# AlanConfluent/flink

Hardware: AMD Instinct MI355X
Metric: records/sec aggregated (1M-key tumbling SUM) (higher is better)
Workload: dtype int64

## Files before the change

flink_amd/csrc/engine.hip:

```cpp
#include <hip/hip_runtime.h>
#include <hipcub/device/device_radix_sort.hpp>
#include <hipcub/device/device_scan.hpp>

#include <algorithm>
#include <cstdio>
#include <cstdlib>
#include <cstring>
#include <map>
#include <set>
#include <string>
#include <vector>

#include "../../include/flink_amd.h"
#include "java_math.h"
#include "dec_view.h"

#define LONG_MIN_J ((int64_t)0x8000000000000000LL)
#define LONG_MAX_J ((int64_t)0x7fffffffffffffffLL)

namespace {

#include "ingest.inc"


// ... 1793 lines not shown
    if (rel2slot) {
        uint8_t* code = (uint8_t*)(rel2slot + kRelCap);
        uint8_t* fresh = code + kRelCap;
        for (int32_t i = t; i < kRelCap; i += nt) {
            const int32_t j = i - tab.lo;
            const bool in = j >= 0 && j < tab.n;
            rel2slot[i] = in ? tab.slot[j] : -1;
            code[i] = in ? tab.code[j] : kCodeSlow;
            fresh[i] = in ? tab.fresh[j] : (uint8_t)0;
        }
    }
    if (t == 0) {
        st->error = 0; st->spill_n = 0; st->want_n = 0; st->key_full = 0;
        st->rows = 0;
        st->dropped = 0; st->late_fire = 0; st->max_q = 0; st->min_q = ~0ull; st->ovf_n = 0; st->strag_n = 0; st->wide_n = 0;
    }
    for (int32_t i = t; i < nwant; i += nt) want[i] = 0ull;
    for (int32_t i = t; i < nbcnt; i += nt) bcnt[i] = 0u;
}

struct SlotList { int32_t n, id[15]; };
__global__ void reset_slots_kernel(unsigned long long* const* slot_base, const int32_t* list, SlotList inl, int64_t stride,
                                   int32_t* touched, const EngineConst* __restrict__ cp) {
    const EngineConst& c = *cp;
    const int32_t sid = inl.n ? inl.id[blockIdx.y] : list[blockIdx.y];
    const int32_t slot = sid < 0 ? ~sid : sid;
    if (sid < 0) {
        if (blockIdx.x == 0 && threadIdx.x == 0) touched[slot] = 0;
        return;
    }
// ... 228 lines not shown
    bool sparse = false;
    bool red = false;
    unsigned long long* d_rk = nullptr;
    int32_t* d_iota = nullptr;
    int64_t iota_cap = 0;
    int64_t iota_n = 0;
    bool iota_pending = false, iota_ran = false;
    int32_t* d_rslots = nullptr;
    int64_t rslots_cap = 0;
    int64_t rk_cap = 0;
    int64_t red_seq_base = 0;
    SpState* sp = nullptr;
    int32_t opt_pre = -1, opt_mp = -1, opt_narrow = -1, opt_cells = -1;
    int32_t opt_variant = 0;
    int64_t stragglers = 0;
    bool rows_zero = false;
    int64_t fused_fires = 0;
    int64_t reset_launches = 0;
    int32_t push_epoch = 0;
    unsigned long long* d_rsum = nullptr;
    bool rs_valid = false;
    int64_t rs_q0 = 0;
    int32_t rs_u0 = 0, rs_epoch = 0;
    int32_t rs_k = 4;
    bool rs_on = true;
    int64_t rs_used = 0;
    int64_t opt_out_min = 0;
    bool opt_partials_v1 = false;
    int32_t opt_profile = 0;
    void* d_mf = nullptr;
// ... 905 lines not shown
        e->d_bval[0] = e->d_bval[1] = nullptr;
        const int64_t ent = capb * e->np * kSub + 8 * kMaxPart;
        HIPCHK(e, hipMalloc(&e->d_bkey, (e->nv == 1 ? 12 : 8) * ent));
        HIPCHK(e, hipMalloc(&e->d_brel, 2 * ent));
        for (int v = 0; v < e->nv; ++v) HIPCHK(e, hipMalloc(&e->d_bval[v], 8 * ent));
        e->capb = capb;
    }
    if (need_bn && !e->d_bn) HIPCHK(e, hipMalloc(&e->d_bn, 2 * (e->capb * e->np * kSub + 8 * kMaxPart)));
    if (!e->d_bcnt) {
        HIPCHK(e, hipMalloc(&e->d_bcnt, sizeof(uint32_t) * kMaxPart * kSub));
        HIPCHK(e, hipMalloc(&e->d_rel2slot, (sizeof(int32_t) + 2) * kRelCap));
    }
    return FWA_OK;
}

static int print_phase_profile(fwa_engine* e, const char* tag, hipEvent_t a, hipEvent_t b, int nb, int nph) {
    HIPCHK(e, hipStreamSynchronize(e->stream));
    float ms = 0.f;
    HIPCHK(e, hipEventElapsedTime(&ms, a, b));
    std::vector<long long> hp(8 * (size_t)nb);
    HIPCHK(e, hipMemcpy(hp.data(), e->d_prof, sizeof(long long) * 8 * nb, hipMemcpyDeviceToHost));
    double tot[8] = {0};
    int bmax = 0;
    long long bsum_max = -1;
    for (int blk = 0; blk < nb; ++blk) {
        long long bs = 0;
        for (int k = 0; k < nph; ++k) { tot[k] += (double)hp[blk * 8 + k] / nb; bs += hp[blk * 8 + k]; }
        if (bs > bsum_max) { bsum_max = bs; bmax = blk; }
    }
    fprintf(stderr, "[%s] kernel %.3f ms; per-block avg cycles:", tag, ms);
    for (int k = 0; k < nph; ++k) fprintf(stderr, " %.0f", tot[k]);
    fprintf(stderr, " | slowest block %d:", bmax);
    for (int k = 0; k < nph; ++k) fprintf(stderr, " %lld", hp[bmax * 8 + k]);
    fprintf(stderr, "\n");
    return FWA_OK;
}

static int ensure_sort_tmp(fwa_engine* e, size_t bytes);
static int push_v2(fwa_engine* e, IngestArgs& a, bool* ran) {
    *ran = false;
    int layout = 0;
    if (e->nacc_comb == 1) layout = 2;
    else if (e->nacc_comb == 2 && e->ec.acc_kind[1] == ACC_ADD_I64) {
        for (int j = 0; j < e->cfg.num_aggs; ++j)
            if (e->ec.agg[j].acc == 1 && e->ec.agg[j].vslot == 0) layout = 1;
    }
    const bool pre_ok = (layout == 2 && e->nv == 0) || (layout == 1 && e->nv == 1 && e->vsize[0] == 8);
    if (a.pcount && (!pre_ok || e->cfg.nullable_cols || e->opt_partials_v1)) return FWA_OK;
// ... 77 lines not shown
    pa.b_val0 = e->d_bval[0];
    pa.b_val1 = e->d_bval[1];
    pa.b_cnt = e->d_bcnt;
    pa.capb = e->capb;
    pa.trash = (uint64_t)e->capb * e->np * kSub;
    pa.spill_cap = e->spill_cap;
    pa.part_bits = e->part_bits;
    pa.np = e->np;
    pa.sub_major = (e->opt_variant & 4) ? 0 : 1;
    pa.iota1 = e->ec.red_iota && e->nv == 2 && e->vcol[1] == kIotaCol && e->vsize[1] == 4 && !(e->opt_variant & 16);
    if (e->iota_pending && !pa.iota1) { int rc = ensure_iota(e); if (rc) return rc; }
    for (int v = 0; v < 2; ++v) { pa.vcol[v] = e->vcol[v]; pa.vsize[v] = e->vsize[v]; }
    pa.dropidx = a.pcount ? nullptr : a.dropidx;
    for (int c = 0; c < FWA_MAX_COLS; ++c) { pa.nulls[c] = a.nulls[c]; pa.any_null |= a.nulls[c] != nullptr; }
    pa.st = e->d_st;
    if (e->opt_profile && !e->d_prof) HIPCHK(e, hipMalloc(&e->d_prof, sizeof(long long) * 8 * kMaxPart));
    pa.prof = e->opt_profile ? e->d_prof : nullptr;
    HIPCHK(e, hipEventRecord(e->ev[4], e->stream));
    const int threads = 1024;
    const int items = e->nv == 2 ? 4 : (e->nv == 1 ? 6 : 8);
    const int64_t tile = (int64_t)items * threads;
    const int grid = (int)std::max<int64_t>(1, std::min<int64_t>((a.n + tile - 1) / tile, 256));
    const int vw = (e->vsize[0] == 8 ? 1 : 0) | (e->vsize[1] == 8 ? 2 : 0);
    const bool kg_all = e->cfg.kg_start == 0 && e->cfg.kg_end == e->cfg.max_parallelism - 1 &&
                        e->cfg.key_kind != FWA_KEY_GROUP_PREFIXED;
    const int kgm = kg_all ? 0 : (e->cfg.key_kind == FWA_KEY_PREHASHED ? 2 : 1);
    auto al16 = [](const void* q) { return q == nullptr || ((uintptr_t)q & 15) == 0; };
    const bool w16 = kgm == 0 && al16(pa.keys) && al16(pa.ts) &&
                     (e->nv == 0 || ((uintptr_t)pa.cols[pa.vcol[0]] & ((e->vsize[0] == 8) ? 15 : 7)) == 0);
    const bool narrow = e->opt_narrow != 0 && (e->opt_narrow == 1 || e->narrow) && layout == 1 && e->nv == 1 &&
                        (vw & 1) && w16 && !pre && !a.pcount;
// ... 56 lines not shown
#define FWA_C3_IT0 4
#endif
#ifndef FWA_C3_IT1
#define FWA_C3_IT1 4
#endif
#ifndef FWA_C3_IT2
#define FWA_C3_IT2 3
#endif
#ifndef FWA_C3_NIT
#define FWA_C3_NIT 6
#endif
#ifndef FWA_MP_IT
#define FWA_MP_IT 2
#endif
    constexpr int TH3 = FWA_C3_TH;
#define C3M(IT, NV, LY, PR) do { if (mp) combine3_kernel<FWA_MP_IT, 2, NV, TH3, LY, PR, 1><<<e->np, TH3, lds3, e->stream>>>(ca, e->d_ec); \
        else combine3_kernel<IT, 2, NV, TH3, LY, PR, 0><<<e->np, TH3, lds3, e->stream>>>(ca, e->d_ec); } while (0)
#define C3L(IT, NV) do { \
        if (pre && layout == 1) C3M(IT, 1, 1, 1); \
        else if (pre) C3M(IT, 0, 2, 1); \
        else if (layout == 1) C3M(IT, NV, 1, 0); \
        else if (layout == 2) C3M(IT, NV, 2, 0); \
        else C3M(IT, NV, 0, 0); } while (0)
    if (narrow) {
        if (mp) combine3_kernel<FWA_MP_IT, 2, 1, TH3, 1, 0, 1, 1><<<e->np, TH3, lds3, e->stream>>>(ca, e->d_ec);
        else if (TH3 != 1024 || (e->opt_variant & 2)) combine3_kernel<FWA_C3_NIT, 2, 1, TH3, 1, 0, 0, 1><<<e->np, TH3, lds3, e->stream>>>(ca, e->d_ec);
        else combine3_kernel<6, 2, 1, 1024, 1, 0, 0, 1, 3><<<e->np, 1024, lds3, e->stream>>>(ca, e->d_ec);
    } else if (narrow2) {
        if (mp) combine3_kernel<FWA_MP_IT, 2, 2, TH3, 0, 0, 1, 2><<<e->np, TH3, lds3, e->stream>>>(ca, e->d_ec);
        else combine3_kernel<4, 2, 2, TH3, 0, 0, 0, 2><<<e->np, TH3, lds3, e->stream>>>(ca, e->d_ec);
    } else if (e->nv == 0) C3L(FWA_C3_IT0, 0);
    else if (e->nv == 1) C3L(FWA_C3_IT1, 1);
    else C3L(FWA_C3_IT2, 2);
#undef C3L
#undef C3M
    HIPCHK(e, hipGetLastError());
    HIPCHK(e, hipEventRecord(e->ev[7], e->stream));
    e->v2_timing_pending = true;
    if (e->opt_profile) {
        int rc2 = print_phase_profile(e, "aprof", e->ev[6], e->ev[7], e->np, 8);
        if (rc2) return rc2;
    }
    e->ingest_launches++;
    e->ingest_records += a.n;
    *ran = true;
    return FWA_OK;
}

struct KidEq {
    int tb;
    __host__ __device__ bool operator()(unsigned long long x, unsigned long long y) const { return (x >> tb) == (y >> tb); }
};
struct MaxI64 {
    __host__ __device__ int64_t operator()(int64_t x, int64_t y) const { return x > y ? x : y; }
};
// ... 759 lines not shown
        if (rc) return rc;
        if (e->v2_timing_pending) {
            float ms = 0.f;
            HIPCHK(e, hipEventElapsedTime(&ms, e->ev[4], e->ev[5]));
            e->partition_ms += ms;
            e->ingest_ms += ms;
            HIPCHK(e, hipEventElapsedTime(&ms, e->ev[6], e->ev[7]));
            e->combine_ms += ms;
            e->ingest_ms += ms;
            e->v2_timing_pending = false;
        }
        if (!ran_v2 || round > 0) { rc = account_ingest(e); if (rc) return rc; }
        const DevStatus st = *e->h_st;
        if (ran_v2 && round == 0 && (int64_t)st.ovf_n * 64 > n) e->pre = true;
        if (ran_v2 && round == 0 && (int64_t)st.strag_n * 64 > n) e->mp = true;
        if (ran_v2 && round == 0) e->stragglers += st.strag_n;
        if (ran_v2 && round == 0 && e->narrow_used && (int64_t)st.wide_n * 64 > n) e->narrow = false;
        if (st.error) {
            const char* m = st.error == FWA_E_KEYGROUP ? "Key group is not in the owned KeyGroupRange (StateTable.getMapForKeyGroup)"
                          : st.error == FWA_E_TS_MIN ? "Record has Long.MIN_VALUE timestamp (= no timestamp marker)."
                          : st.error == FWA_E_OOM ? (st.key_full ? "key table full: raise fwa_config.key_capacity" : "slice want-set overflow")
                                                  : "device error";
            return fail(e, st.error, m);
        }
        if (st.late_fire) {
            const size_t o = late_idx.size();
            late_idx.resize(o + st.late_fire);
            HIPCHK(e, hipMemcpy(late_idx.data() + o, e->d_late, 4 * (size_t)st.late_fire, hipMemcpyDeviceToHost));
        }
        dropped += (int64_t)st.dropped;
        if (st.max_q) qmax = std::max<int64_t>(qmax, jm::unord_i64(st.max_q));
// ... 1443 lines not shown
        case FWA_OPT_PARTIALS_ONE_PASS: e->opt_partials_v1 = value > 0; return FWA_OK;
        case FWA_OPT_SP_TABLE: case FWA_OPT_SP_FMAX: case FWA_OPT_SP_BUDGET: return sp_set_option(e, option, value);
        case FWA_OPT_PROFILE: e->opt_profile = value > 0 ? 1 : 0; return FWA_OK;
        case FWA_OPT_INGEST_VARIANT: e->opt_variant = (int32_t)std::max<int64_t>(0, value); return FWA_OK;
        case FWA_OPT_SLIDE_CARRIED: e->rs_on = value != 0; e->rs_valid = false; return FWA_OK;
        case FWA_OPT_FIRE_PARTIALS: e->opt_fire_partials = value != 0 ? 1 : 0; return FWA_OK;
        case FWA_OPT_DEC_WRAP_NULL: e->opt_dec_wrap_null = value != 0 ? 1 : 0; return FWA_OK;
        case FWA_OPT_DISTINCT_SLOTS:
            if (!e->dist) return fail(e, FWA_E_UNSUPPORTED, "FWA_OPT_DISTINCT_SLOTS: no COUNT(DISTINCT) aggregate");
            if (e->dist->d_tab) return fail(e, FWA_E_STATE, "FWA_OPT_DISTINCT_SLOTS: before the first push");
            if (value < 64 || (value & (value - 1)) || value > ((int64_t)1 << 40))
                return fail(e, FWA_E_ARG, "FWA_OPT_DISTINCT_SLOTS: a power of two >= 64");
            e->dist->first_slots = value;
            return FWA_OK;
        case FWA_OPT_DISTINCT_LIVE: case FWA_OPT_DISTINCT_REBUILDS: case FWA_OPT_STRAGGLERS: case FWA_OPT_KEY_TABLE_DIGEST:
        case FWA_OPT_DISTINCT_INDEX_US: case FWA_OPT_DISTINCT_COUNT_US: case FWA_OPT_DISTINCT_COUNT_STEPS:
            return fail(e, FWA_E_ARG, "read-only option");
        default: return fail(e, FWA_E_ARG, "unknown option");
    }
}

int fwa_get_option(const fwa_engine* e, int32_t option, int64_t* value) {
    if (!e || !value) return FWA_E_ARG;
    auto eff = [](int32_t opt, bool adaptive_on) -> int64_t { return opt == 1 || (opt != 0 && adaptive_on) ? 1 : 0; };
    switch (option) {
        case FWA_OPT_SKEW_MERGE: *value = eff(e->opt_pre, e->pre); return FWA_OK;
        case FWA_OPT_WINDOW_PASSES: *value = eff(e->opt_mp, e->mp); return FWA_OK;
        case FWA_OPT_NARROW_ENTRIES: *value = eff(e->opt_narrow, e->narrow); return FWA_OK;
        case FWA_OPT_SESSION_CELLS: *value = eff(e->opt_cells, e->cell_skip <= 0); return FWA_OK;
        case FWA_OPT_OUT_MIN_ROWS: *value = e->opt_out_min > 0 ? e->opt_out_min : ((int64_t)1 << 22); return FWA_OK;
        case FWA_OPT_PARTIALS_ONE_PASS: *value = e->opt_partials_v1 ? 1 : 0; return FWA_OK;
        case FWA_OPT_SP_TABLE: case FWA_OPT_SP_FMAX: case FWA_OPT_SP_BUDGET:
            if (!e->sp) return FWA_E_UNSUPPORTED;
            *value = option == FWA_OPT_SP_TABLE ? e->sp->T : option == FWA_OPT_SP_FMAX ? (e->sp->fmax ? e->sp->fmax : kSpMaxF)
                                                                                    : (int64_t)e->sp->budget;
            return FWA_OK;
        case FWA_OPT_PROFILE: *value = e->opt_profile; return FWA_OK;
        case FWA_OPT_SESSION_PATH: *value = e->sess_path; return FWA_OK;
        case FWA_OPT_INGEST_VARIANT: *value = e->opt_variant; return FWA_OK;
        case FWA_OPT_SLIDE_CARRIED: *value = e->rs_used; return FWA_OK;
        case FWA_OPT_FIRE_PARTIALS: *value = e->mf_calls - e->mf_fallbacks; return FWA_OK;
        case FWA_OPT_DEC_WRAP_NULL: *value = e->opt_dec_wrap_null; return FWA_OK;
        case FWA_OPT_FUSED_FIRES: *value = e->fused_fires; return FWA_OK;
        case FWA_OPT_RESET_LAUNCHES: *value = e->reset_launches; return FWA_OK;
        case FWA_OPT_STRAGGLERS: *value = e->stragglers; return FWA_OK;
        case FWA_OPT_KEY_TABLE_DIGEST: {
            std::vector<unsigned long long> table((size_t)e->capacity + 1);
            if (!e->d_keys || hipStreamSynchronize(e->stream) != hipSuccess ||
                hipMemcpy(table.data(), e->d_keys, 8 * table.size(), hipMemcpyDeviceToHost) != hipSuccess) return FWA_E_DEVICE;
            uint64_t h = 0xcbf29ce484222325ull;
            for (unsigned long long w : table)
                for (int b = 0; b < 8; ++b) h = (h ^ ((w >> (8 * b)) & 0xff)) * 0x100000001b3ull;
            *value = (int64_t)h;
            return FWA_OK;
        }
        case FWA_OPT_DISTINCT_SLOTS: case FWA_OPT_DISTINCT_LIVE: case FWA_OPT_DISTINCT_REBUILDS:
            if (!e->dist) return FWA_E_UNSUPPORTED;
            *value = option == FWA_OPT_DISTINCT_SLOTS ? (e->dist->slots ? e->dist->slots : e->dist->first_slots)
                   : option == FWA_OPT_DISTINCT_LIVE ? e->dist->live : e->dist->rebuilds;
            return FWA_OK;
// ... 54 lines not shown
```

flink_amd/csrc/ingest.inc:

```

#ifdef FWA_KPROF
#define KPROF(p) ((p) != nullptr)
#else
#define KPROF(p) false
#endif

constexpr int kBlock = 256;
constexpr uint64_t kEmptyKey = 0x8000000000000000ull;
constexpr int kBucket = 8;
constexpr int32_t kWantCap = 1 << 14;


struct DirEntry {
    int64_t q;
    int32_t slot;
    int32_t flags;
    int64_t thr;
    int64_t first_maxts;
};

struct DevStatus {
    int32_t error;
    int32_t spill_n;
    int32_t want_n;
    int32_t key_full;
    unsigned long long dropped;
    unsigned long long n_keys;
    unsigned long long late_fire;
    unsigned long long rows;
    unsigned long long max_q;
    unsigned long long min_q;
    int32_t pad;
    int32_t pad2;
    unsigned long long sess_live;
    unsigned long long drop_n;
    int32_t ovf_n;
    int32_t strag_n;
    int32_t wide_n;
    int32_t pad3;
};

__device__ __forceinline__ void note_drop(int32_t* list, DevStatus* st, bool drop, int64_t i) {
    if (!list) return;
    const unsigned long long m = __ballot(drop);
    if (!m) return;
    const int lane = threadIdx.x & 63;
    const int ld = __ffsll((long long)m) - 1;
    unsigned long long b = 0;
    if (lane == ld) b = atomicAdd(&st->drop_n, (unsigned long long)__popcll(m));
    b = __shfl(b, ld);
    if (drop) list[b + __popcll(m & ((1ull << lane) - 1))] = (int32_t)i;
}

// ... 778 lines not shown
constexpr int kStragL = 256;
struct StragL {
    uint32_t g, n;
    int32_t rel, pad;
    unsigned long long x0, x1;
};

__device__ __forceinline__ uint32_t kswz(uint32_t s) { return s ^ (((s >> 5) & 3u) << 1); }


typedef __attribute__((address_space(1))) unsigned long long g_u64;
typedef const __attribute__((address_space(1))) unsigned long long* gc_u64_ptr;

constexpr int32_t kLeanEmpty = (int32_t)0x80000000;
constexpr int32_t kLeanForeign = (int32_t)0x80000001;
typedef int32_t lean_i4 __attribute__((ext_vector_type(4)));

__device__ __forceinline__ uint32_t kswz32(uint32_t s) { return s ^ (((s >> 6) & 1u) << 2); }

__device__ __forceinline__ int32_t lean_key_image(unsigned long long k) {
    if (k == kEmptyKey) return kLeanEmpty;
    const bool narrow = (int64_t)(int32_t)(uint32_t)k == (int64_t)k && (uint32_t)k - 0x80000000u > 1u;
    return narrow ? (int32_t)(uint32_t)k : kLeanForeign;
}

template <int BT>
__device__ __forceinline__ void lean_pin(const lean_i4* qa, const lean_i4* qb) {
    static_assert(BT >= 1 && BT <= 4, "batch size");
    if constexpr (BT == 1) asm volatile("" : : "v"(qa[0]), "v"(qb[0]));
    else if constexpr (BT == 2) asm volatile("" : : "v"(qa[0]), "v"(qb[0]), "v"(qa[1]), "v"(qb[1]));
// ... 40 lines not shown
    const uint32_t h = z2lo ^ ((z2lo >> 31) | (z2hi << 1));
    return h & smask & ~(uint32_t)(kBucket - 1);
}

template <bool kMax>
__device__ __forceinline__ int lean_wave_red(int v) {
    auto step = [](int x, int y) { return kMax ? max(x, y) : (int)min((uint32_t)x, (uint32_t)y); };
    v = step(v, __builtin_amdgcn_update_dpp(0, v, 0xB1, 0xf, 0xf, true));
    v = step(v, __builtin_amdgcn_update_dpp(0, v, 0x4E, 0xf, 0xf, true));
    v = step(v, __builtin_amdgcn_update_dpp(0, v, 0x141, 0xf, 0xf, true));
    v = step(v, __builtin_amdgcn_update_dpp(0, v, 0x140, 0xf, 0xf, true));
    return step(step(__builtin_amdgcn_readlane(v, 0), __builtin_amdgcn_readlane(v, 16)),
                step(__builtin_amdgcn_readlane(v, 32), __builtin_amdgcn_readlane(v, 48)));
}

template <int IT, int BT, int SL, int TH>
__device__ __forceinline__ void combine3_lean(const CombineArgs& a, const EngineConst& c) {
    extern __shared__ __attribute__((aligned(16))) unsigned char smem[];
    static_assert(IT % BT == 0, "whole batches");
    static_assert(TH / kSub == 64, "one wave per sub-bucket");
    constexpr int kWaves = TH / 64;
    const int tid = threadIdx.x, lane = tid & 63, wv = tid >> 6;
    const int p = blockIdx.x;
    const int seg = 1 << a.seg_log;
    const uint32_t smask = (uint32_t)seg - 1u;
    __shared__ StragL s_strag[kStragL];
    __shared__ int s_sn;
    int32_t* lkey = (int32_t*)smem;
    uint32_t* lcnt = (uint32_t*)(smem + (size_t)seg * 8);
    unsigned long long* lacc = (unsigned long long*)(smem + (size_t)seg * 8 + (size_t)SL * seg * 4);
    int* s_mm = (int*)(smem + (size_t)seg * 8 + (size_t)SL * seg * 4 + (size_t)SL * seg * 8);
    int* s_new = s_mm + 4 * kWaves;
    long long pt = clock64();
    long long pacc[8] = {0, 0, 0, 0, 0, 0, 0, 0};
#define PMARK(k) do { if (KPROF(a.prof)) { const long long _t = clock64(); pacc[k] += _t - pt; pt = _t; } } while (0)
    unsigned long long* gkeys = a.key_table + ((int64_t)p << a.seg_log);
    for (int i = tid; i < seg; i += TH) lkey[kswz32((uint32_t)i)] = lean_key_image(gkeys[i]);
    for (int i = tid; i < SL * seg; i += TH) { lcnt[i] = 0; lacc[i] = 0ull; }
    if (tid == 0) { *s_new = 0; s_sn = 0; }
    if (tid < 3) { s_mm[2 * tid] = 0x7fffffff; s_mm[2 * tid + 1] = -1; }
    constexpr int64_t kChunk = (int64_t)IT * 64;
    const int my_cnt = __builtin_amdgcn_readfirstlane((int)min((int64_t)a.b_cnt[p * kSub + wv], a.capb));
    const int64_t boff = (int64_t)bucket_base(p, wv, a.np, a.sub_major) * a.capb;
    int64_t cnt = 0;
    for (int s2 = 0; s2 < kSub; ++s2) cnt = max(cnt, min((int64_t)a.b_cnt[p * kSub + s2], a.capb));
    const gc_u64_ptr bk = (const gc_u64_ptr)(a.b_key + boff);
    const __attribute__((address_space(1))) uint16_t* br = (const __attribute__((address_space(1))) uint16_t*)(a.b_rel + boff);
    int lo = 0x7fffffff;
    auto flush = [&](int rel) {
        constexpr int kPer = 4096 / TH;
        const int w = rel & (SL - 1);
        const int32_t slot = (rel >= 0 && rel < kRelCap) ? a.rel2slot[rel] : -1;
        g_u64* base = slot >= 0 ? (g_u64*)a.slot_base[slot] : nullptr;
        const bool fresh = slot >= 0 && a.relfresh && a.relfresh[rel];
// ... 7 lines not shown
            g[m] = ((int64_t)p << a.seg_log) + i;
            if (i < seg) { k[m] = lcnt[w * seg + i]; lcnt[w * seg + i] = 0; }
            if (k[m]) { x[m] = lacc[(size_t)w * seg + i]; lacc[(size_t)w * seg + i] = 0ull; }
        }
        if (!base) return;
        g_u64* col = base + a.stride;
        unsigned long long old[kPer], old1[kPer];
#pragma unroll
        for (int m = 0; m < kPer; ++m) {
            old[m] = (k[m] && !fresh) ? base[g[m]] : 0ull;
            old1[m] = (k[m] && !fresh) ? col[g[m]] : 0ull;
        }
#pragma unroll
        for (int m = 0; m < kPer; ++m) if (k[m]) { base[g[m]] = old[m] + k[m]; col[g[m]] = old1[m] + x[m]; }
    };
    __syncthreads();
    unsigned long long nkey[IT];
    int nrel[IT];
    auto load_chunk = [&](int64_t cb) {
        if (cb + kChunk <= (int64_t)my_cnt) {
            const gc_u64_ptr pk = bk + cb + lane;
            const __attribute__((address_space(1))) uint16_t* pr = br + cb + lane;
#pragma unroll
            for (int j = 0; j < IT; ++j) { nkey[j] = pk[j * 64]; nrel[j] = (int)pr[j * 64]; }
        } else {
#pragma unroll
            for (int j = 0; j < IT; ++j) {
                const int64_t i = cb + (int64_t)j * 64 + lane;
                const bool ok = i < (int64_t)my_cnt;
                nkey[j] = ok ? bk[i] : 0ull;
// ... 25 lines not shown
        if (lane == 0) { atomicMin(&mm[0], wmin); atomicMax(&mm[1], wmax); }
        if (tid == 0) { int* nx = s_mm + 2 * ((it + 1) % 3); nx[0] = 0x7fffffff; nx[1] = -1; }
        uint32_t hb[IT];
#pragma unroll
        for (int j = 0; j < IT; ++j) {
            hb[j] = lean_home(key[j], smask);
            consume(hb[j]);
        }
        PMARK(2);
        __syncthreads();
        PMARK(3);
        const int cmin = __builtin_amdgcn_readfirstlane(mm[0]), cmax = __builtin_amdgcn_readfirstlane(mm[1]);
        if (cmax < 0) continue;
        if (lo == 0x7fffffff) lo = cmin;
        if (cmax >= lo + SL) {
            while (cmax >= lo + SL) { flush(lo); ++lo; if (KPROF(a.prof)) pacc[7] += 1000; }
            __syncthreads();
        }
        const int lo_c = lo;
        PMARK(4);
        if (KPROF(a.prof)) pacc[7] += 1;
        uint32_t miss = 0;
#pragma unroll
        for (int j0 = IT - BT; j0 >= 0; j0 -= BT) {
            lean_i4 qa[BT], qb[BT];
#pragma unroll
            for (int u = 0; u < BT; ++u) {
                qa[u] = *(const lean_i4*)&lkey[hb[j0 + u]];
                qb[u] = *(const lean_i4*)&lkey[hb[j0 + u] + 4];
            }
// ... 1 lines not shown
#pragma unroll
            for (int u = BT - 1; u >= 0; --u) {
                const int32_t t = lean_match(qa[u], qb[u], key[j0 + u]);
                const uint32_t b = hb[j0 + u];
                hb[j0 + u] = b + (((uint32_t)t ^ (b >> 4)) & 4u) + ((uint32_t)t & 3u);
                miss = __builtin_amdgcn_alignbit(miss, (uint32_t)t, 31);
            }
        }
        uint32_t todo = miss;
        if (!whole) {
            uint32_t ok = 0;
#pragma unroll
            for (int j = 0; j < IT; ++j) ok |= rel[j] >= 0 ? (1u << j) : 0u;
            todo &= ok;
        }
        while (todo) {
            const int jm_ = __builtin_ctz(todo);
            todo &= todo - 1u;
            int32_t kk = key[0];
            uint32_t b = hb[0];
#pragma unroll
            for (int j = 1; j < IT; ++j) { kk = jm_ == j ? key[j] : kk; b = jm_ == j ? hb[j] : b; }
            b &= ~(uint32_t)(kBucket - 1);
            int32_t found = -1;
            for (int round = 0; round <= (seg >> 2) && found < 0; ++round) {
                const uint32_t f = ((b >> 6) & 1u) << 2;
                const lean_i4 pa = *(const lean_i4*)&lkey[b + f];
                const lean_i4 pb = *(const lean_i4*)&lkey[b + (f ^ 4u)];
                const int32_t eq = lean_match(pa, pb, kk), em = lean_match(pa, pb, kLeanEmpty);
                if (eq >= 0) { found = (int32_t)(b + (uint32_t)eq); break; }
                if (em >= 0) {
                    const uint32_t sidx = b + (uint32_t)em;
                    const int32_t old = atomicCAS(&lkey[kswz32(sidx)], kLeanEmpty, kk);
                    if (old == kLeanEmpty) { found = (int32_t)sidx; atomicAdd(s_new, 1); break; }
                    if (old == kk) { found = (int32_t)sidx; break; }
                    continue;
                }
                b = (b + kBucket) & smask;
            }
            if (found >= 0) miss &= ~(1u << jm_);
#pragma unroll
            for (int j = 0; j < IT; ++j) hb[j] = (jm_ == j && found >= 0) ? (uint32_t)found : hb[j];
        }
        uint32_t out = 0;
#pragma unroll
        for (int j = 0; j < IT; ++j) out |= (uint32_t)(rel[j] - lo_c) & ~(uint32_t)(SL - 1);
        if (__builtin_amdgcn_ballot_w64((out | miss) != 0u) == 0ull) {
#pragma unroll
            for (int j = 0; j < IT; ++j) {
                const uint32_t at = ((uint32_t)(rel[j] & (SL - 1)) << a.seg_log) + hb[j];
                atomicAdd(&lcnt[at], 1u);
                atomicAdd(&lacc[at], (unsigned long long)(int64_t)val[j]);
            }
        } else {
#pragma unroll
            for (int j = 0; j < IT; ++j) {
                if (rel[j] < 0 || rel[j] >= lo + SL) continue;
                if (miss & (1u << j)) { a.st->key_full = 1; raise_error(a.st, FWA_E_OOM); continue; }
                const int32_t local = (int32_t)hb[j];
                const unsigned long long x0 = (unsigned long long)(int64_t)val[j];
                if (rel[j] < lo_c) {
                    if (KPROF(a.prof)) pacc[6] += 1000000;
                    const uint32_t g = (uint32_t)(((int64_t)p << a.seg_log) + local);
                    const int si = atomicAdd(&s_sn, 1);
                    if (si < kStragL) s_strag[si] = StragL{g, 1u, rel[j], 0, x0, 0ull};
                    else strag_apply(a, c, rel[j], g, 1u, x0, 0ull);
                    continue;
                }
                const int w = rel[j] & (SL - 1);
                atomicAdd(&lcnt[w * seg + local], 1u);
                atomicAdd(&lacc[(size_t)w * seg + local], x0);
            }
        }
        PMARK(5);
    }
    __syncthreads();
    if (lo != 0x7fffffff)
        for (int r = lo; r < lo + SL; ++r) flush(r);
    __syncthreads();
    if (tid == 0 && s_sn) atomicAdd(&a.st->strag_n, s_sn);
    for (int t = tid; t < min(s_sn, kStragL); t += TH) {
        const StragL se = s_strag[t];
        strag_apply(a, c, se.rel, se.g, se.n, se.x0, se.x1);
    }
    if (*s_new) {
        for (int i = tid; i < seg; i += TH) {
            const int32_t k32 = lkey[kswz32((uint32_t)i)];
            if (k32 != kLeanEmpty && gkeys[i] == kEmptyKey) gkeys[i] = (unsigned long long)(int64_t)k32;
        }
        if (tid == 0) atomicAdd(&a.st->n_keys, (unsigned long long)*s_new);
    }
    if (KPROF(a.prof) && tid == 0) for (int q = 0; q < 8; ++q) a.prof[(int64_t)p * 8 + q] = pacc[q];
#undef PMARK
}

template <int IT, int SL, int NV, int TH, int LAYOUT, int PRE = 0, int MP = 0, int NW = 0, int LEAN = 0>
__global__ void __launch_bounds__(TH, 1) combine3_kernel(CombineArgs a, const EngineConst* __restrict__ cp) {
    if constexpr (LEAN != 0) {
        static_assert(NW == 1 && LAYOUT == 1 && NV == 1 && PRE == 0 && MP == 0, "lean body: narrow COUNT + SUM entries");
        combine3_lean<IT, LEAN, SL, TH>(a, *cp);
        return;
    }
    extern __shared__ __attribute__((aligned(16))) unsigned char smem[];
    constexpr int kWaves = TH / 64;
    constexpr int LPS = TH / kSub;
    static_assert(LPS == 32 || LPS == 64, "sub-bucket lane mapping");
    const EngineConst& c = *cp;
    const int tid = threadIdx.x, lane = tid & 63, wv = tid >> 6;
    const int sub = tid / LPS, li = tid % LPS;
    const int p = blockIdx.x;
    const int seg = 1 << a.seg_log;
    const uint32_t smask = (uint32_t)seg - 1u;
    const int nacc = LAYOUT == 1 ? 2 : (LAYOUT == 2 ? 1 : c.nacc_comb);
    __shared__ int s_desc[kMaxAggsInt + 1];
    __shared__ StragL s_strag[kStragL];
// ... 262 lines not shown
```

flink_amd/engine.py:

```python
import ctypes as C
import os

import numpy as np

from . import _abi as A

_HERE = os.path.dirname(os.path.abspath(__file__))
LIB_PATH = os.path.join(_HERE, "libflink_amd.so")
_LIB = None


class EngineError(RuntimeError):
    def __init__(self, code, msg):
        super().__init__("%s: %s" % (A.STATUS.get(code, code), msg))
        self.code = code


class Blob(C.Structure):
    _fields_ = [("data", C.c_void_p), ("size", C.c_int64)]


def lib():
    global _LIB
    if _LIB is not None:
# ... 103 lines not shown
                raise ValueError("%s: %s columns beside %s keys" % (name, "CUDA" if not device else "host",
                                                                     "CUDA" if device else "host"))


def _check(rc, h=None, what=""):
    if rc:
        msg = lib().fwa_last_error(h).decode() if h else what
        raise EngineError(rc, msg or what)


OPTIONS = {"skew_merge": 1, "window_passes": 2, "narrow_entries": 3, "session_cells": 4, "out_min_rows": 5,
           "partials_one_pass": 6, "sp_table": 7, "sp_fmax": 8, "sp_budget": 9, "profile": 10,
           "session_path": 11, "ingest_variant": 12, "slide_carried": 13, "fire_partials": 14, "dec_wrap_null": 15,
           "fused_fires": 16, "reset_launches": 17, "distinct_slots": 18, "distinct_live": 19, "distinct_rebuilds": 20,
           "stragglers": 21, "key_table_digest": 22, "distinct_index_us": 23, "distinct_count_us": 24,
           "distinct_count_steps": 25}
DEFAULT_OPTIONS = {}


class WindowAggregator:

    def __init__(self, cfg, options=None):
        self.cfg = cfg
        self.names = A.agg_names(cfg)
        self.h = C.c_void_p()
        self._inflight = None
        self._in_stream = None
        rc = lib().fwa_create(C.byref(cfg), C.byref(self.h))
        if rc:
            why = lib().fwa_last_error(None).decode()
            raise EngineError(rc, "fwa_create" + (": " + why if why and why != "null engine" else ""))
# ... 372 lines not shown
```

include/flink_amd.h:

```cpp
#ifndef FLINK_AMD_H
#define FLINK_AMD_H

#include <stdint.h>

#ifdef __cplusplus
extern "C" {
#endif

#define FWA_ABI_VERSION 5
#define FWA_MAX_AGGS 8
#define FWA_MAX_COLS 8

enum fwa_window_kind { FWA_TUMBLE = 0, FWA_SLIDE = 1, FWA_CUMULATE = 2, FWA_SESSION = 3 };

enum fwa_semantics { FWA_SEM_DATASTREAM = 0, FWA_SEM_TABLE = 1 };

enum fwa_key_kind { FWA_KEY_JAVA_LONG = 0, FWA_KEY_BINROW_BIGINT = 1, FWA_KEY_PREHASHED = 2,
                    FWA_KEY_GROUP_PREFIXED = 3  };

enum fwa_agg_kind {
    FWA_COUNT = 0,
    FWA_SUM_I64 = 1,
    FWA_SUM_F32 = 2,
    FWA_SUM_F64 = 3,
// ... 208 lines not shown
    FWA_OPT_PROFILE = 10,
    FWA_OPT_SESSION_PATH = 11,
    FWA_OPT_INGEST_VARIANT = 12,
    FWA_OPT_SLIDE_CARRIED = 13,
    FWA_OPT_FIRE_PARTIALS = 14,
    FWA_OPT_DEC_WRAP_NULL = 15,
    FWA_OPT_FUSED_FIRES = 16,
    FWA_OPT_RESET_LAUNCHES = 17,
    FWA_OPT_DISTINCT_SLOTS = 18,
    FWA_OPT_DISTINCT_LIVE = 19,
    FWA_OPT_DISTINCT_REBUILDS = 20,
    FWA_OPT_STRAGGLERS = 21,
    FWA_OPT_KEY_TABLE_DIGEST = 22,
    FWA_OPT_DISTINCT_INDEX_US = 23,
    FWA_OPT_DISTINCT_COUNT_US = 24,
    FWA_OPT_DISTINCT_COUNT_STEPS = 25
};
int fwa_set_option(fwa_engine* e, int32_t option, int64_t value);
int fwa_get_option(const fwa_engine* e, int32_t option, int64_t* value);

int fwa_key_groups(const int64_t* keys, const int32_t* key_hash, int64_t n, int32_t key_kind,
                   int32_t max_parallelism, int32_t parallelism, int32_t* kg_out, int32_t* op_out,
                   int32_t flags, int32_t device);

int fwa_route_rows(const int64_t* keys, const int32_t* key_hash, int64_t n, int32_t key_kind, int32_t max_parallelism,
                   int32_t parallelism, const void* const* cols, const int32_t* col_bytes, int32_t ncols, int64_t* out,
                   int64_t* counts, int32_t device, void* stream);

int fwa_unpack_rows(const int64_t* rows, int64_t n, int32_t ncols, int64_t* const* cols, int32_t device, void* stream);

enum fwa_key_field_type { FWA_KEY_FIELD_BIGINT = 0, FWA_KEY_FIELD_INT = 1, FWA_KEY_FIELD_DOUBLE = 2,
// ... 40 lines not shown
```

Measured before the change: 61.61 billion.

## Queue hash-probe misses in LDS and drain them block-wide in lean combine

Result: no change. 61.79 billion (median of 6 runs) (+0.3%).

```diff
diff --git a/flink_amd/csrc/engine.hip b/flink_amd/csrc/engine.hip
--- a/flink_amd/csrc/engine.hip
+++ b/flink_amd/csrc/engine.hip
@@ -1831,6 +1831,7 @@
         st->error = 0; st->spill_n = 0; st->want_n = 0; st->key_full = 0;
         st->rows = 0;
         st->dropped = 0; st->late_fire = 0; st->max_q = 0; st->min_q = ~0ull; st->ovf_n = 0; st->strag_n = 0; st->wide_n = 0;
+        st->missq_n = 0; st->missd_n = 0;
     }
     for (int32_t i = t; i < nwant; i += nt) want[i] = 0ull;
     for (int32_t i = t; i < nbcnt; i += nt) bcnt[i] = 0u;
@@ -2089,6 +2090,7 @@
     int32_t opt_pre = -1, opt_mp = -1, opt_narrow = -1, opt_cells = -1;
     int32_t opt_variant = 0;
     int64_t stragglers = 0;
+    int64_t miss_queued = 0, miss_direct = 0;
     bool rows_zero = false;
     int64_t fused_fires = 0;
     int64_t reset_launches = 0;
@@ -3024,24 +3026,25 @@
     return FWA_OK;
 }
 
-static int print_phase_profile(fwa_engine* e, const char* tag, hipEvent_t a, hipEvent_t b, int nb, int nph) {
+constexpr int kProfRowMax = 10;
+static int print_phase_profile(fwa_engine* e, const char* tag, hipEvent_t a, hipEvent_t b, int nb, int nph, int row = 8) {
     HIPCHK(e, hipStreamSynchronize(e->stream));
     float ms = 0.f;
     HIPCHK(e, hipEventElapsedTime(&ms, a, b));
-    std::vector<long long> hp(8 * (size_t)nb);
-    HIPCHK(e, hipMemcpy(hp.data(), e->d_prof, sizeof(long long) * 8 * nb, hipMemcpyDeviceToHost));
-    double tot[8] = {0};
+    std::vector<long long> hp((size_t)row * nb);
+    HIPCHK(e, hipMemcpy(hp.data(), e->d_prof, sizeof(long long) * row * nb, hipMemcpyDeviceToHost));
+    double tot[kProfRowMax] = {0};
     int bmax = 0;
     long long bsum_max = -1;
     for (int blk = 0; blk < nb; ++blk) {
         long long bs = 0;
-        for (int k = 0; k < nph; ++k) { tot[k] += (double)hp[blk * 8 + k] / nb; bs += hp[blk * 8 + k]; }
+        for (int k = 0; k < nph; ++k) { tot[k] += (double)hp[blk * row + k] / nb; bs += hp[blk * row + k]; }
         if (bs > bsum_max) { bsum_max = bs; bmax = blk; }
     }
     fprintf(stderr, "[%s] kernel %.3f ms; per-block avg cycles:", tag, ms);
     for (int k = 0; k < nph; ++k) fprintf(stderr, " %.0f", tot[k]);
     fprintf(stderr, " | slowest block %d:", bmax);
-    for (int k = 0; k < nph; ++k) fprintf(stderr, " %lld", hp[bmax * 8 + k]);
+    for (int k = 0; k < nph; ++k) fprintf(stderr, " %lld", hp[bmax * row + k]);
     fprintf(stderr, "\n");
     return FWA_OK;
 }
@@ -3149,7 +3152,7 @@
     pa.dropidx = a.pcount ? nullptr : a.dropidx;
     for (int c = 0; c < FWA_MAX_COLS; ++c) { pa.nulls[c] = a.nulls[c]; pa.any_null |= a.nulls[c] != nullptr; }
     pa.st = e->d_st;
-    if (e->opt_profile && !e->d_prof) HIPCHK(e, hipMalloc(&e->d_prof, sizeof(long long) * 8 * kMaxPart));
+    if (e->opt_profile && !e->d_prof) HIPCHK(e, hipMalloc(&e->d_prof, sizeof(long long) * kProfRowMax * kMaxPart));
     pa.prof = e->opt_profile ? e->d_prof : nullptr;
     HIPCHK(e, hipEventRecord(e->ev[4], e->stream));
     const int threads = 1024;
@@ -3236,6 +3239,7 @@
 #define FWA_MP_IT 2
 #endif
     constexpr int TH3 = FWA_C3_TH;
+    bool lean = false;
 #define C3M(IT, NV, LY, PR) do { if (mp) combine3_kernel<FWA_MP_IT, 2, NV, TH3, LY, PR, 1><<<e->np, TH3, lds3, e->stream>>>(ca, e->d_ec); \
         else combine3_kernel<IT, 2, NV, TH3, LY, PR, 0><<<e->np, TH3, lds3, e->stream>>>(ca, e->d_ec); } while (0)
 #define C3L(IT, NV) do { \
@@ -3247,7 +3251,8 @@
     if (narrow) {
         if (mp) combine3_kernel<FWA_MP_IT, 2, 1, TH3, 1, 0, 1, 1><<<e->np, TH3, lds3, e->stream>>>(ca, e->d_ec);
         else if (TH3 != 1024 || (e->opt_variant & 2)) combine3_kernel<FWA_C3_NIT, 2, 1, TH3, 1, 0, 0, 1><<<e->np, TH3, lds3, e->stream>>>(ca, e->d_ec);
-        else combine3_kernel<6, 2, 1, 1024, 1, 0, 0, 1, 3><<<e->np, 1024, lds3, e->stream>>>(ca, e->d_ec);
+        else if (e->opt_variant & 512) { combine3_kernel<6, 2, 1, 1024, 1, 0, 0, 1, 3, 0><<<e->np, 1024, lds3, e->stream>>>(ca, e->d_ec); lean = true; }
+        else { combine3_kernel<6, 2, 1, 1024, 1, 0, 0, 1, 3, 1><<<e->np, 1024, lds3, e->stream>>>(ca, e->d_ec); lean = true; }
     } else if (narrow2) {
         if (mp) combine3_kernel<FWA_MP_IT, 2, 2, TH3, 0, 0, 1, 2><<<e->np, TH3, lds3, e->stream>>>(ca, e->d_ec);
         else combine3_kernel<4, 2, 2, TH3, 0, 0, 0, 2><<<e->np, TH3, lds3, e->stream>>>(ca, e->d_ec);
@@ -3260,7 +3265,8 @@
     HIPCHK(e, hipEventRecord(e->ev[7], e->stream));
     e->v2_timing_pending = true;
     if (e->opt_profile) {
-        int rc2 = print_phase_profile(e, "aprof", e->ev[6], e->ev[7], e->np, 8);
+        int rc2 = lean ? print_phase_profile(e, "aprof", e->ev[6], e->ev[7], e->np, kLeanProf, kLeanProf)
+                       : print_phase_profile(e, "aprof", e->ev[6], e->ev[7], e->np, 8);
         if (rc2) return rc2;
     }
     e->ingest_launches++;
@@ -4050,7 +4056,7 @@
         const DevStatus st = *e->h_st;
         if (ran_v2 && round == 0 && (int64_t)st.ovf_n * 64 > n) e->pre = true;
         if (ran_v2 && round == 0 && (int64_t)st.strag_n * 64 > n) e->mp = true;
-        if (ran_v2 && round == 0) e->stragglers += st.strag_n;
+        if (ran_v2 && round == 0) { e->stragglers += st.strag_n; e->miss_queued += st.missq_n; e->miss_direct += st.missd_n; }
         if (ran_v2 && round == 0 && e->narrow_used && (int64_t)st.wide_n * 64 > n) e->narrow = false;
         if (st.error) {
             const char* m = st.error == FWA_E_KEYGROUP ? "Key group is not in the owned KeyGroupRange (StateTable.getMapForKeyGroup)"
@@ -5524,6 +5530,7 @@
             e->dist->first_slots = value;
             return FWA_OK;
         case FWA_OPT_DISTINCT_LIVE: case FWA_OPT_DISTINCT_REBUILDS: case FWA_OPT_STRAGGLERS: case FWA_OPT_KEY_TABLE_DIGEST:
+        case FWA_OPT_MISS_QUEUED: case FWA_OPT_MISS_DIRECT:
         case FWA_OPT_DISTINCT_INDEX_US: case FWA_OPT_DISTINCT_COUNT_US: case FWA_OPT_DISTINCT_COUNT_STEPS:
             return fail(e, FWA_E_ARG, "read-only option");
         default: return fail(e, FWA_E_ARG, "unknown option");
@@ -5554,6 +5561,8 @@
         case FWA_OPT_FUSED_FIRES: *value = e->fused_fires; return FWA_OK;
         case FWA_OPT_RESET_LAUNCHES: *value = e->reset_launches; return FWA_OK;
         case FWA_OPT_STRAGGLERS: *value = e->stragglers; return FWA_OK;
+        case FWA_OPT_MISS_QUEUED: *value = e->miss_queued; return FWA_OK;
+        case FWA_OPT_MISS_DIRECT: *value = e->miss_direct; return FWA_OK;
         case FWA_OPT_KEY_TABLE_DIGEST: {
             std::vector<unsigned long long> table((size_t)e->capacity + 1);
             if (!e->d_keys || hipStreamSynchronize(e->stream) != hipSuccess ||
diff --git a/flink_amd/csrc/ingest.inc b/flink_amd/csrc/ingest.inc
--- a/flink_amd/csrc/ingest.inc
+++ b/flink_amd/csrc/ingest.inc
@@ -37,6 +37,8 @@
     int32_t ovf_n;
     int32_t strag_n;
     int32_t wide_n;
+    int32_t missq_n;
+    int32_t missd_n;
     int32_t pad3;
 };
 
@@ -845,6 +847,7 @@
 
 constexpr int32_t kLeanEmpty = (int32_t)0x80000000;
 constexpr int32_t kLeanForeign = (int32_t)0x80000001;
+constexpr int kLeanProf = 10;
 typedef int32_t lean_i4 __attribute__((ext_vector_type(4)));
 
 __device__ __forceinline__ uint32_t kswz32(uint32_t s) { return s ^ (((s >> 6) & 1u) << 2); }
@@ -915,7 +918,26 @@
                 step(__builtin_amdgcn_readlane(v, 32), __builtin_amdgcn_readlane(v, 48)));
 }
 
-template <int IT, int BT, int SL, int TH>
+__device__ __forceinline__ int32_t lean_probe(int32_t* lkey, uint32_t b, int32_t kk, uint32_t smask, int seg, int* s_new) {
+    for (int round = 0; round <= (seg >> 2); ++round) {
+        const uint32_t f = ((b >> 6) & 1u) << 2;
+        const lean_i4 pa = *(const lean_i4*)&lkey[b + f];
+        const lean_i4 pb = *(const lean_i4*)&lkey[b + (f ^ 4u)];
+        const int32_t eq = lean_match(pa, pb, kk), em = lean_match(pa, pb, kLeanEmpty);
+        if (eq >= 0) return (int32_t)(b + (uint32_t)eq);
+        if (em >= 0) {
+            const uint32_t sidx = b + (uint32_t)em;
+            const int32_t old = atomicCAS(&lkey[kswz32(sidx)], kLeanEmpty, kk);
+            if (old == kLeanEmpty) { atomicAdd(s_new, 1); return (int32_t)sidx; }
+            if (old == kk) return (int32_t)sidx;
+            continue;
+        }
+        b = (b + kBucket) & smask;
+    }
+    return -1;
+}
+
+template <int IT, int BT, int SL, int TH, int MQ>
 __device__ __forceinline__ void combine3_lean(const CombineArgs& a, const EngineConst& c) {
     extern __shared__ __attribute__((aligned(16))) unsigned char smem[];
     static_assert(IT % BT == 0, "whole batches");
@@ -932,13 +954,17 @@
     unsigned long long* lacc = (unsigned long long*)(smem + (size_t)seg * 8 + (size_t)SL * seg * 4);
     int* s_mm = (int*)(smem + (size_t)seg * 8 + (size_t)SL * seg * 4 + (size_t)SL * seg * 8);
     int* s_new = s_mm + 4 * kWaves;
+    __shared__ int s_q[3];
+    const int qcap = MQ && seg * 4 / 10 >= 64 ? seg * 4 / 10 : 0;
+    unsigned long long* qw = (unsigned long long*)(smem + (size_t)seg * 4);
+    uint16_t* qr = (uint16_t*)(smem + (size_t)seg * 4 + (size_t)qcap * 8);
     long long pt = clock64();
-    long long pacc[8] = {0, 0, 0, 0, 0, 0, 0, 0};
+    long long pacc[kLeanProf] = {0, 0, 0, 0, 0, 0, 0, 0, 0, 0};
 #define PMARK(k) do { if (KPROF(a.prof)) { const long long _t = clock64(); pacc[k] += _t - pt; pt = _t; } } while (0)
     unsigned long long* gkeys = a.key_table + ((int64_t)p << a.seg_log);
     for (int i = tid; i < seg; i += TH) lkey[kswz32((uint32_t)i)] = lean_key_image(gkeys[i]);
     for (int i = tid; i < SL * seg; i += TH) { lcnt[i] = 0; lacc[i] = 0ull; }
-    if (tid == 0) { *s_new = 0; s_sn = 0; }
+    if (tid == 0) { *s_new = 0; s_sn = 0; s_q[0] = 0; s_q[1] = 0; s_q[2] = 0; }
     if (tid < 3) { s_mm[2 * tid] = 0x7fffffff; s_mm[2 * tid + 1] = -1; }
     constexpr int64_t kChunk = (int64_t)IT * 64;
     const int my_cnt = __builtin_amdgcn_readfirstlane((int)min((int64_t)a.b_cnt[p * kSub + wv], a.capb));
@@ -976,6 +1002,38 @@
 #pragma unroll
         for (int m = 0; m < kPer; ++m) if (k[m]) { base[g[m]] = old[m] + k[m]; col[g[m]] = old1[m] + x[m]; }
     };
+    auto apply_missed = [&](int32_t kk, int32_t v, int r, int lo_c) {
+        const int32_t local = lean_probe(lkey, lean_home(kk, smask), kk, smask, seg, s_new);
+        if (r >= lo_c + SL) return;
+        if (local < 0) { a.st->key_full = 1; raise_error(a.st, FWA_E_OOM); return; }
+        const unsigned long long x0 = (unsigned long long)(int64_t)v;
+        if (r < lo_c) {
+            if (KPROF(a.prof)) pacc[6] += 1000000;
+            const uint32_t g = (uint32_t)(((int64_t)p << a.seg_log) + local);
+            const int si = atomicAdd(&s_sn, 1);
+            if (si < kStragL) s_strag[si] = StragL{g, 1u, r, 0, x0, 0ull};
+            else strag_apply(a, c, r, g, 1u, x0, 0ull);
+            return;
+        }
+        const int w = r & (SL - 1);
+        atomicAdd(&lcnt[w * seg + local], 1u);
+        atomicAdd(&lacc[(size_t)w * seg + local], x0);
+    };
+    auto drain = [&](int lo_c) {
+        const int n = min(s_q[0], qcap);
+        for (int i = tid; i < n; i += TH) {
+            const unsigned long long w = qw[i];
+            apply_missed((int32_t)(uint32_t)w, (int32_t)(uint32_t)(w >> 32), (int)qr[i], lo_c);
+        }
+    };
+    auto drain_done = [&]() {
+        if (tid == 0) {
+            const int t = s_q[0];
+            s_q[1] += min(t, qcap);
+            s_q[2] += max(t - qcap, 0);
+            s_q[0] = 0;
+        }
+    };
     __syncthreads();
     unsigned long long nkey[IT];
     int nrel[IT];
@@ -1031,6 +1089,11 @@
         if (cmax < 0) continue;
         if (lo == 0x7fffffff) lo = cmin;
         if (cmax >= lo + SL) {
+            if constexpr (MQ != 0) {
+                drain(lo);
+                __syncthreads();
+                drain_done();
+            }
             while (cmax >= lo + SL) { flush(lo); ++lo; if (KPROF(a.prof)) pacc[7] += 1000; }
             __syncthreads();
         }
@@ -1062,6 +1125,36 @@
             for (int j = 0; j < IT; ++j) ok |= rel[j] >= 0 ? (1u << j) : 0u;
             todo &= ok;
         }
+        PMARK(5);
+        uint32_t queued = 0;
+        if constexpr (MQ != 0) {
+            if (__builtin_amdgcn_ballot_w64(todo != 0u) != 0ull) {
+                unsigned long long mj[IT];
+                int tot = 0;
+#pragma unroll
+                for (int j = 0; j < IT; ++j) {
+                    mj[j] = __builtin_amdgcn_ballot_w64(((todo >> j) & 1u) != 0u);
+                    tot += __popcll(mj[j]);
+                }
+                int base = 0;
+                if (lane == 0) base = atomicAdd(&s_q[0], tot);
+                base = __builtin_amdgcn_readfirstlane(base);
+#pragma unroll
+                for (int j = 0; j < IT; ++j) {
+                    if (mj[j] == 0ull) continue;
+                    const int pos = base + (int)__builtin_amdgcn_mbcnt_hi((uint32_t)(mj[j] >> 32),
+                                                                          __builtin_amdgcn_mbcnt_lo((uint32_t)mj[j], 0u));
+                    if (((todo >> j) & 1u) != 0u && pos < qcap) {
+                        qw[pos] = (unsigned long long)(uint32_t)key[j] | ((unsigned long long)(uint32_t)val[j] << 32);
+                        qr[pos] = (uint16_t)rel[j];
+                        val[j] = 0;
+                        queued |= 1u << j;
+                    }
+                    base += __popcll(mj[j]);
+                }
+                todo &= ~queued;
+            }
+        }
         while (todo) {
             const int jm_ = __builtin_ctz(todo);
             todo &= todo - 1u;
@@ -1069,41 +1162,28 @@
             uint32_t b = hb[0];
 #pragma unroll
             for (int j = 1; j < IT; ++j) { kk = jm_ == j ? key[j] : kk; b = jm_ == j ? hb[j] : b; }
-            b &= ~(uint32_t)(kBucket - 1);
-            int32_t found = -1;
-            for (int round = 0; round <= (seg >> 2) && found < 0; ++round) {
-                const uint32_t f = ((b >> 6) & 1u) << 2;
-                const lean_i4 pa = *(const lean_i4*)&lkey[b + f];
-                const lean_i4 pb = *(const lean_i4*)&lkey[b + (f ^ 4u)];
-                const int32_t eq = lean_match(pa, pb, kk), em = lean_match(pa, pb, kLeanEmpty);
-                if (eq >= 0) { found = (int32_t)(b + (uint32_t)eq); break; }
-                if (em >= 0) {
-                    const uint32_t sidx = b + (uint32_t)em;
-                    const int32_t old = atomicCAS(&lkey[kswz32(sidx)], kLeanEmpty, kk);
-                    if (old == kLeanEmpty) { found = (int32_t)sidx; atomicAdd(s_new, 1); break; }
-                    if (old == kk) { found = (int32_t)sidx; break; }
-                    continue;
-                }
-                b = (b + kBucket) & smask;
-            }
+            const int32_t found = lean_probe(lkey, b & ~(uint32_t)(kBucket - 1), kk, smask, seg, s_new);
             if (found >= 0) miss &= ~(1u << jm_);
 #pragma unroll
             for (int j = 0; j < IT; ++j) hb[j] = (jm_ == j && found >= 0) ? (uint32_t)found : hb[j];
         }
+        PMARK(8);
         uint32_t out = 0;
 #pragma unroll
         for (int j = 0; j < IT; ++j) out |= (uint32_t)(rel[j] - lo_c) & ~(uint32_t)(SL - 1);
-        if (__builtin_amdgcn_ballot_w64((out | miss) != 0u) == 0ull) {
+        if (__builtin_amdgcn_ballot_w64((out | (miss & ~queued)) != 0u) == 0ull) {
+            const uint32_t live = ~queued;
 #pragma unroll
             for (int j = 0; j < IT; ++j) {
                 const uint32_t at = ((uint32_t)(rel[j] & (SL - 1)) << a.seg_log) + hb[j];
-                atomicAdd(&lcnt[at], 1u);
+                atomicAdd(&lcnt[at], MQ != 0 ? (live >> j) & 1u : 1u);
                 atomicAdd(&lacc[at], (unsigned long long)(int64_t)val[j]);
             }
         } else {
 #pragma unroll
             for (int j = 0; j < IT; ++j) {
                 if (rel[j] < 0 || rel[j] >= lo + SL) continue;
+                if (queued & (1u << j)) continue;
                 if (miss & (1u << j)) { a.st->key_full = 1; raise_error(a.st, FWA_E_OOM); continue; }
                 const int32_t local = (int32_t)hb[j];
                 const unsigned long long x0 = (unsigned long long)(int64_t)val[j];
@@ -1120,13 +1200,22 @@
                 atomicAdd(&lacc[(size_t)w * seg + local], x0);
             }
         }
-        PMARK(5);
+        PMARK(9);
     }
     __syncthreads();
+    if constexpr (MQ != 0) {
+        drain(lo);
+        __syncthreads();
+        drain_done();
+    }
     if (lo != 0x7fffffff)
         for (int r = lo; r < lo + SL; ++r) flush(r);
     __syncthreads();
     if (tid == 0 && s_sn) atomicAdd(&a.st->strag_n, s_sn);
+    if (MQ != 0 && tid == 0) {
+        if (s_q[1]) atomicAdd(&a.st->missq_n, s_q[1]);
+        if (s_q[2]) atomicAdd(&a.st->missd_n, s_q[2]);
+    }
     for (int t = tid; t < min(s_sn, kStragL); t += TH) {
         const StragL se = s_strag[t];
         strag_apply(a, c, se.rel, se.g, se.n, se.x0, se.x1);
@@ -1138,15 +1227,15 @@
         }
         if (tid == 0) atomicAdd(&a.st->n_keys, (unsigned long long)*s_new);
     }
-    if (KPROF(a.prof) && tid == 0) for (int q = 0; q < 8; ++q) a.prof[(int64_t)p * 8 + q] = pacc[q];
+    if (KPROF(a.prof) && tid == 0) for (int q = 0; q < kLeanProf; ++q) a.prof[(int64_t)p * kLeanProf + q] = pacc[q];
 #undef PMARK
 }
 
-template <int IT, int SL, int NV, int TH, int LAYOUT, int PRE = 0, int MP = 0, int NW = 0, int LEAN = 0>
+template <int IT, int SL, int NV, int TH, int LAYOUT, int PRE = 0, int MP = 0, int NW = 0, int LEAN = 0, int MQ = 0>
 __global__ void __launch_bounds__(TH, 1) combine3_kernel(CombineArgs a, const EngineConst* __restrict__ cp) {
     if constexpr (LEAN != 0) {
         static_assert(NW == 1 && LAYOUT == 1 && NV == 1 && PRE == 0 && MP == 0, "lean body: narrow COUNT + SUM entries");
-        combine3_lean<IT, LEAN, SL, TH>(a, *cp);
+        combine3_lean<IT, LEAN, SL, TH, MQ>(a, *cp);
         return;
     }
     extern __shared__ __attribute__((aligned(16))) unsigned char smem[];
diff --git a/flink_amd/engine.py b/flink_amd/engine.py
--- a/flink_amd/engine.py
+++ b/flink_amd/engine.py
@@ -141,7 +141,7 @@
            "session_path": 11, "ingest_variant": 12, "slide_carried": 13, "fire_partials": 14, "dec_wrap_null": 15,
            "fused_fires": 16, "reset_launches": 17, "distinct_slots": 18, "distinct_live": 19, "distinct_rebuilds": 20,
            "stragglers": 21, "key_table_digest": 22, "distinct_index_us": 23, "distinct_count_us": 24,
-           "distinct_count_steps": 25}
+           "distinct_count_steps": 25, "miss_queued": 26, "miss_direct": 27}
 DEFAULT_OPTIONS = {}
 
 
diff --git a/include/flink_amd.h b/include/flink_amd.h
--- a/include/flink_amd.h
+++ b/include/flink_amd.h
@@ -246,7 +246,9 @@
     FWA_OPT_KEY_TABLE_DIGEST = 22,
     FWA_OPT_DISTINCT_INDEX_US = 23,
     FWA_OPT_DISTINCT_COUNT_US = 24,
-    FWA_OPT_DISTINCT_COUNT_STEPS = 25
+    FWA_OPT_DISTINCT_COUNT_STEPS = 25,
+    FWA_OPT_MISS_QUEUED = 26,
+    FWA_OPT_MISS_DIRECT = 27
 };
 int fwa_set_option(fwa_engine* e, int32_t option, int64_t value);
 int fwa_get_option(const fwa_engine* e, int32_t option, int64_t* value);
```
